# Yusheng-Xu/VGS-SVGS-Segmentation

Measured on AMD Instinct MI355X. Metric: segmented points/sec (end-to-end VGS), higher is better.
Workload: dtype f32

## Files before the change

### vgs-svgs-segmentation_amd/csrc/capi.hip

```cpp
#include <algorithm>
#include <cstdio>
#include <cstdlib>
#include <cstring>
#include <fstream>
#include <string>
#include <vector>

#include <dlfcn.h>

#include "vgs_context.hpp"

static thread_local std::string g_create_err;

static const char* const VGS_STAGE_NAMES[VGS_T_COUNT] = {"vgs:voxelize", "vgs:features", "vgs:adjacency", "vgs:localcut", "vgs:merge", "vgs:labels",
                                                         "vgs:total", "vgs:localcut_kernel", "vgs:supervoxels", "vgs:localcut_bulk", "", ""};
struct RoctxApi {
  int (*push)(const char*) = nullptr;
  int (*pop)() = nullptr;
  RoctxApi() {
    for (const char* name : {"librocprofiler-sdk-roctx.so.1", "librocprofiler-sdk-roctx.so", "libroctx64.so.4", "libroctx64.so"}) {
      void* h = dlopen(name, RTLD_LAZY | RTLD_LOCAL);
      if (!h) continue;
      push = (int (*)(const char*))dlsym(h, "roctxRangePushA");
      pop = (int (*)())dlsym(h, "roctxRangePop");
// ... 132 lines not shown
  }
  if (p->device < 0 || p->device >= ndev) { g_create_err = "vgs_create: bad device ordinal"; return VGS_E_ARG; }
  vgs_ctx* c = new (std::nothrow) vgs_ctx();
  if (!c) return VGS_E_NOMEM;
  c->P = *p;
  c->device = p->device;
  int prio_lo = 0, prio_hi = 0;
  if (hipSetDevice(c->device) != hipSuccess || hipStreamCreateWithFlags(&c->stream, hipStreamNonBlocking) != hipSuccess ||
      hipDeviceGetStreamPriorityRange(&prio_lo, &prio_hi) != hipSuccess ||
      hipStreamCreateWithPriority(&c->stream2, hipStreamNonBlocking, prio_hi) != hipSuccess ||
      hipStreamCreateWithPriority(&c->stream3, hipStreamNonBlocking, prio_hi) != hipSuccess ||
      hipStreamCreateWithPriority(&c->stream4, hipStreamNonBlocking, prio_hi) != hipSuccess) {
    g_create_err = "vgs_create: hipSetDevice/hipStreamCreate failed";
    vgs_destroy(c);
    return VGS_E_HIP;
  }
  if (hipHostMalloc(&c->pin, 4096, hipHostMallocDefault) != hipSuccess) c->pin = nullptr;
  bool ok = hipStreamCreateWithFlags(&c->s_h2d, hipStreamNonBlocking) == hipSuccess &&
            hipStreamCreateWithFlags(&c->s_d2h, hipStreamNonBlocking) == hipSuccess &&
            hipEventCreateWithFlags(&c->ev_h2d, hipEventDisableTiming) == hipSuccess &&
            hipEventCreateWithFlags(&c->ev_d2h, hipEventDisableTiming) == hipSuccess &&
            hipEventCreateWithFlags(&c->ev_rb, hipEventDisableTiming) == hipSuccess &&
            hipEventCreateWithFlags(&c->ev_ho, hipEventDisableTiming) == hipSuccess &&
            hipEventCreateWithFlags(&c->ev_ho2, hipEventDisableTiming) == hipSuccess;
  for (int i = 0; ok && i < 16; ++i) ok = hipEventCreate(&c->ev[i]) == hipSuccess;
  for (int i = 0; ok && i < VGS_T_COUNT; ++i) ok = hipEventCreate(&c->tev[i][0]) == hipSuccess && hipEventCreate(&c->tev[i][1]) == hipSuccess;
  if (!ok) { g_create_err = "vgs_create: hipStreamCreate/hipEventCreate failed"; vgs_destroy(c); return VGS_E_HIP; }
  vgs_read_env_knobs(c);
  *out = c;
  return VGS_OK;
}

void vgs_destroy(vgs_ctx* c) {
  if (!c) return;
  (void)hipSetDevice(c->device);
  if (c->stream) (void)hipStreamSynchronize(c->stream);
  if (c->stream2) (void)hipStreamSynchronize(c->stream2);
  if (c->stream3) (void)hipStreamSynchronize(c->stream3);
  if (c->stream4) (void)hipStreamSynchronize(c->stream4);
  if (c->s_h2d) (void)hipStreamSynchronize(c->s_h2d);
  if (c->s_d2h) (void)hipStreamSynchronize(c->s_d2h);
  c->xyz_buf[0].release(); c->xyz_buf[1].release(); c->pt_label_alt.release(); c->grow_state.release();
  c->code_a.release(); c->code_b.release(); c->perm_a.release(); c->perm_b.release(); c->sort_tmp.release();
  c->head_flag.release(); c->pt_vox.release(); c->vox_tile.release(); c->vox_code.release(); c->vox_start.release();
  c->xs.release(); c->ys.release(); c->zs.release();
  c->node.release(); c->used_ids.release(); c->used_rank.release();
  c->hkey.release(); c->hval.release(); c->offsets.release(); c->adj_masks.release(); c->adj_gtab.release(); c->adj_nvals.release(); c->adj_nrank.release(); c->adj_key.release(); c->adj_off.release(); c->adj_cnt.release(); c->adj_mused.release();
// ... 15 lines not shown
  c->ps_in.release(); c->ps_nnodes.release(); c->ps_key.release(); c->ps_val.release(); c->ps_seg.release(); c->ps_nn.release(); c->ps_tmp.release();
  c->ps_meta.release(); c->ps_part.release(); c->ps_d.release(); c->ps_f.release(); c->ps_npts.release();
  c->cl_off.release(); c->cl_idx.release(); c->conn.release(); c->evals.release(); c->lc_pending.release(); c->lc_defer.release(); c->lc_defer_flag.release(); c->csize.release(); c->attach.release(); c->cc_flags.release(); c->parent.release(); c->csz.release();
  c->vc_cen.release(); c->vc_nrm.release(); c->vc_dist.release(); c->vc_state.release(); c->vc_tile_start.release(); c->vc_cell.release(); c->vc_plive.release(); c->vc_tile_of.release(); c->vc_tchg.release(); c->vc_nbr_tiles.release(); c->vc_halo.release(); c->vc_tile_meta.release(); c->vc_pool.release(); c->vc_ring.release(); c->vc_dbg.release(); c->vc_label.release();
  c->vc_seedkey.release(); c->vc_sums.release(); c->vc_count.release(); c->vc_accu.release(); c->vc_alive.release();
  c->sv_label.release(); c->sv_key_a.release(); c->sv_key_b.release(); c->cell_code_a.release(); c->cell_code_b.release();
  c->cell_id_a.release(); c->cell_id_b.release(); c->cell_start.release();
  c->owned.release(); c->straddle.release(); c->mixsrc.release(); c->bnd_code.release(); c->bnd_root.release(); c->root_label.release();
  c->bnd_code2.release(); c->bnd_root2.release(); c->bnd_cnt.release(); c->broot.release();
  c->kept_rank.release(); c->vox_label.release(); c->pt_label.release(); c->counters.release(); c->work_ids.release();
  if (c->pin) (void)hipHostFree(c->pin);
  for (int i = 0; i < 16; ++i) if (c->ev[i]) (void)hipEventDestroy(c->ev[i]);
  for (int i = 0; i < VGS_T_COUNT; ++i) for (int k = 0; k < 2; ++k) if (c->tev[i][k]) (void)hipEventDestroy(c->tev[i][k]);
  if (c->stream) (void)hipStreamDestroy(c->stream);
  if (c->stream2) (void)hipStreamDestroy(c->stream2);
  if (c->stream3) (void)hipStreamDestroy(c->stream3);
  if (c->stream4) (void)hipStreamDestroy(c->stream4);
  if (c->s_h2d) (void)hipStreamDestroy(c->s_h2d);
  if (c->s_d2h) (void)hipStreamDestroy(c->s_d2h);
  if (c->ev_h2d) (void)hipEventDestroy(c->ev_h2d);
  if (c->ev_rb) (void)hipEventDestroy(c->ev_rb);
  if (c->ev_ho) (void)hipEventDestroy(c->ev_ho);
  if (c->ev_ho2) (void)hipEventDestroy(c->ev_ho2);
  if (c->ev_d2h) (void)hipEventDestroy(c->ev_d2h);
  delete c;
}

vgs_status vgs_set_params(vgs_ctx* c, const vgs_params* p) {
  if (!c || !p) return VGS_E_ARG;
  if (!(p->voxel_size > 0.f) || !(p->graph_size > 0.f) || !(p->sig_w != 0.f)) { c->err = "vgs_set_params: voxel_size, graph_size > 0, sig_w != 0"; return VGS_E_ARG; }
  if (p->method != c->P.method || p->device != c->P.device) { c->err = "vgs_set_params: method and device are fixed at vgs_create"; return VGS_E_ARG; }
  if (p->vccs_mode != 0 && p->vccs_mode != 1) { c->err = "vgs_set_params: vccs_mode must be 0 (synchronous variant) or 1 (PCL's order)"; return VGS_E_ARG; }
  int keep = ST_SEGMENTED;
  const vgs_params& o = c->P;
  if (p->cut_thred != o.cut_thred || p->sig_p != o.sig_p || p->sig_n != o.sig_n || p->sig_o != o.sig_o || p->sig_e != o.sig_e ||
      p->sig_c != o.sig_c || p->sig_w != o.sig_w || p->adjacency_min != o.adjacency_min || p->voxels_min != o.voxels_min ||
      p->q7_count_as_index != o.q7_count_as_index)
    keep = ST_ADJACENCY;
  if (p->graph_size != o.graph_size) keep = ST_FEATURES;
  if (p->points_min != o.points_min) keep = ST_VOXELS;
  if (p->voxel_size != o.voxel_size || p->seed_size != o.seed_size || p->color_impt != o.color_impt ||
      p->spatial_impt != o.spatial_impt || p->normal_impt != o.normal_impt || p->vccs_mode != o.vccs_mode)
    keep = ST_POINTS;
  if (c->stage > keep) c->stage = keep;
  if (keep < ST_SEGMENTED) { c->sd_valid = false; c->sb_valid[0] = c->sb_valid[1] = false; c->sg_valid = false; c->cmp_valid = false; c->rf_valid = false; c->cmp_own_cells = -1; c->sg_halo_valid = false; c->sg_own_K = -1; c->rf_halo_valid = false; c->rf_band_n = -1; }
  if (keep == ST_POINTS && c->P.method == 3 && !c->sv_labels_external) { c->sv_have_labels = false; c->sv_max_label = 0; c->sv_label_n = -1; }
// ... 549 lines not shown
```

### vgs-svgs-segmentation_amd/csrc/localcut.hip

```cpp
#include <algorithm>
#include <cmath>
#include <cstring>
#include <vector>
#include <cstdio>
#include <cstdlib>

#include "vgs_context.hpp"

#ifndef LC_TB
#define LC_TB 256
#endif
#ifndef LC_SMALL_CAP
#define LC_SMALL_CAP 4096
#endif
#define LC_NBIN 2048

#define LC_TBINS 64
struct LcParams {
  VgsWeightParams W;
  float cut;
  int prune_unused;
  float d2_stop;
  float ctab_scale;
  const float* ctab;
// ... 789 lines not shown
      const size_t sm = lc_smem_bytes<SMALL_M, SMALL_CAP, false>();
      VGS_HIP_TRY(c, hipFuncSetAttribute((const void*)kern, hipFuncAttributeMaxDynamicSharedMemorySize, (int)sm));
      hipLaunchKernelGGL(kern, dim3(nw), dim3(LC_TB), sm, strm, ids, arg_n, n_dev, c->adj_key.p, c->adj_cnt.p, c->adj_stride,
                         c->node.p, LP, c->conn.p, cnt, c->evals.p, (uint32_t*)nullptr);
    } else {
      auto kern = k_localcut<LARGE_M, LARGE_CAP, false>;
      const size_t sm = lc_smem_bytes<LARGE_M, LARGE_CAP, false>();
      VGS_HIP_TRY(c, hipFuncSetAttribute((const void*)kern, hipFuncAttributeMaxDynamicSharedMemorySize, (int)sm));
      hipLaunchKernelGGL(kern, dim3(nw), dim3(LC_TB), sm, strm, ids, arg_n, n_dev, c->adj_key.p, c->adj_cnt.p, c->adj_stride,
                         c->node.p, LP, c->conn.p, cnt, c->evals.p, ids_d );
    }
    return VGS_OK;
  };
  static_assert(WAVE_B <= SMALL_M, "wave-kernel hand-overs must fit the mid-size workgroup kernel");
  uint32_t* dbg_buf = nullptr;
#ifdef VGS_PROF
  VGS_HIP_TRY(c, s_dbg.ensure(4 * (size_t)U));
  VGS_HIP_TRY(c, hipMemset(s_dbg.p, 0, 16 * (size_t)U));
  dbg_buf = s_dbg.p;
#endif
  VGS_HIP_TRY(c, hipEventRecord(c->ev[6], c->stream));
  if (WP.dbg_stop != 0 || WP.shell0 < 0.0f) VGS_HIP_TRY(c, hipMemsetAsync(c->conn.p, 0, (size_t)U * c->adj_stride, c->stream));
  c->pl_enabled_at_launch = false;
  c->lc_tail.gated = false; c->lc_tail.pg_xl_queued = false;
  c->lc_tail.open = true; c->lc_tail.dense = dense; c->lc_tail.grid_f = 0; c->lc_tail.grid_g = GRID_G; c->lc_tail.tail_ms = 0.f;
  VGS_HIP_TRY(c, hipEventRecord(c->ev[2], c->stream));
  VGS_HIP_TRY(c, hipStreamWaitEvent(c->stream2, c->ev[2], 0));
  VGS_HIP_TRY(c, hipStreamWaitEvent(c->stream3, c->ev[2], 0));
  VGS_HIP_TRY(c, hipEventRecord(c->ev[9], c->stream3));
  VGS_HIP_TRY(c, hipStreamWaitEvent(c->stream, c->ev[9], 0));
  const unsigned int n_wide = nabc[2] + nabc[3] + nabc[5];
  bool pg_wide = c->pl_enabled && c->K.pg_wide != 0 && dense && n_wide > 0 && (uint64_t)n_wide * (uint64_t)c->K.pg_wide_frac > (uint64_t)U;
  if (pg_wide) {
    VGS_HIP_TRY(c, hipStreamWaitEvent(c->stream4, c->ev[2], 0));
    vgs_status sb = vgs_pairlists_build(c, c->stream2, nullptr, nullptr, nullptr, 0, true, LP.ctab, LP.ctab_scale, LP.d2_stop, 0, LcGate{nullptr, 0u}, true);
    if (sb != VGS_OK) return sb;
    pg_wide = c->pl_enabled;
  }
  if (pg_wide) {
    const PairLists PLw = {(const uint2*)c->pl_state.p, c->pl_ent.p, c->pl_state.p + (size_t)c->V * 9, c->pl_w_ring};
    const PgGeom G = {c->vox_code.p, c->P.voxel_size, (float)c->box.min[0], (float)c->box.min[1], (float)c->box.min[2], c->adj_r2};
    uint32_t* const wbits = c->cb_enabled ? c->conn_bits.p : (uint32_t*)nullptr;
    uint32_t* const ids_xl_pg = c->work_ids.p + (10 + LW_HO_BINS) * U;
    unsigned int* const d_nxl = (unsigned int*)(c->counters.p + 56);
    const bool pg_xl = c->cb_R <= 10 && !c->K.no_pg_xl && n_above_d != 0u;
    c->lc_tail.pg_xl_queued = pg_xl && nabc[3] > 0;
    VGS_HIP_TRY(c, hipEventRecord(c->ev_ho2, c->stream2));
// ... 125 lines not shown
  }
  VGS_HIP_TRY(c, hipStreamWaitEvent(c->stream, c->ev[8], 0));
  VGS_HIP_TRY(c, hipStreamWaitEvent(c->stream, c->ev[5], 0));
  if (nabc[3] + nabc[5] > 0) VGS_HIP_TRY(c, hipStreamWaitEvent(c->stream, c->ev[12], 0));
  if (c->K.no_overlap) {
    VGS_HIP_TRY(c, hipStreamWaitEvent(c->stream, c->ev[4], 0));
    VGS_HIP_TRY(c, hipStreamWaitEvent(c->stream, c->ev[3], 0));
    if (c->cb_enabled)
      hipLaunchKernelGGL(k_conn_bits, dim3((unsigned)U), dim3(64), 0, c->stream, c->lc_pending.p, U, c->adj_cnt.p, c->adj_stride, c->conn.p, c->adj_off.p,
                         c->cb_R, c->cb_words, c->conn_bits.p, CbLists{}, 0);
    VGS_HIP_TRY(c, hipMemsetAsync(c->lc_pending.p, 0, (size_t)U, c->stream));
  }
  if (c->pl_enabled_at_launch) c->lc_tail.gated = true;
  c->lc_tail.grid_f = grid_f;
  for (int k = 0; k < 5; ++k) c->lc_tail.nabc[k] = nabc[k];
  c->lc_tail.nabc[2] += nabc[5];
  VGS_HIP_TRY(c, hipEventRecord(c->ev[13], c->stream));
  c->counts[13] = nabc[0] + nabc[4]; c->counts[14] = nabc[1] + nabc[2] + nabc[5] + nabc[6]; c->counts[15] = nabc[3];
  c->counts[VGS_N_PAIRS] = -1;
  VGS_HIP_TRY(c, hipGetLastError());
  return VGS_OK;
}

vgs_status vgs_localcut_finish(vgs_ctx* c, unsigned int* n_deferred) {
  if (n_deferred) *n_deferred = 0;
  if (!c->lc_tail.open) return VGS_OK;
  c->lc_tail.open = false;
  const int64_t U = c->U;
  unsigned long long* cnt = (unsigned long long*)c->counters.p;
  const unsigned int grid_f = c->lc_tail.grid_f, GRID_G = c->lc_tail.grid_g;
  uint32_t* ids_f = c->work_ids.p + 8 * U;
  uint32_t* ids_g = c->work_ids.p + 5 * U;
  LcParams LP;
  LP.W = make_weight_params(c->P);
  LP.cut = c->P.cut_thred;
  LP.prune_unused = 0;
  LP.xl_from = c->K.dbg_xl_from;
  LP.dbg_max_m = c->K.dbg_max_m;
  {
    const float reach = 2.0f * c->P.graph_size + 4.0f * c->P.voxel_size;
    LP.d2_stop = lc_d2_stop(LP.W, LP.cut, reach * reach * 1.01f);
    LP.ctab = c->lc_ctab.p; LP.ctab_scale = c->lc_ctab_scale;
  }
  constexpr int SMALL_M = 128, SMALL_CAP = LC_SMALL_CAP;
  constexpr int LARGE_M = 2048, LARGE_CAP = 8192;
  constexpr int XL_M = 8192, XL_CAP = 4096;
  uint32_t* ids_xl = c->work_ids.p + 3 * U;
  auto launch_rest = [&](const uint32_t* ids, unsigned int nw, bool mid) -> vgs_status {
    if (nw == 0) return VGS_OK;
    if (mid) {
      auto kern = k_localcut<SMALL_M, SMALL_CAP, false>;
      const size_t sm = lc_smem_bytes<SMALL_M, SMALL_CAP, false>();
      VGS_HIP_TRY(c, hipFuncSetAttribute((const void*)kern, hipFuncAttributeMaxDynamicSharedMemorySize, (int)sm));
      hipLaunchKernelGGL(kern, dim3(nw), dim3(LC_TB), sm, c->stream, ids, (int)nw, (const unsigned int*)nullptr, c->adj_key.p, c->adj_cnt.p,
                         c->adj_stride, c->node.p, LP, c->conn.p, cnt, c->evals.p, (uint32_t*)nullptr);
    } else {
      auto kern = k_localcut<LARGE_M, LARGE_CAP, false>;
      const size_t sm = lc_smem_bytes<LARGE_M, LARGE_CAP, false>();
      VGS_HIP_TRY(c, hipFuncSetAttribute((const void*)kern, hipFuncAttributeMaxDynamicSharedMemorySize, (int)sm));
      hipLaunchKernelGGL(kern, dim3(nw), dim3(LC_TB), sm, c->stream, ids, (int)nw, (const unsigned int*)nullptr, c->adj_key.p, c->adj_cnt.p,
                         c->adj_stride, c->node.p, LP, c->conn.p, cnt, c->evals.p, ids_xl);
    }
    return VGS_OK;
  };
  VGS_HIP_TRY(c, hipStreamWaitEvent(c->stream, c->ev[4], 0));
  VGS_HIP_TRY(c, hipStreamWaitEvent(c->stream, c->ev[3], 0));
  VGS_HIP_TRY(c, hipEventRecord(c->ev[7], c->stream));
  unsigned long long hc[64] = {0};
  VGS_READBACK(c, hc, cnt, sizeof(hc));
  const unsigned long long lc_why[4] = {hc[3], hc[4], hc[5], hc[6]};
  if (!c->lc_tail.pg_xl_queued && (unsigned int)(hc[56] & 0xffffffffull) != 0u) { c->err = "local cut: voxels queued for a kernel that was not launched"; return VGS_E_STATE; }
  c->lc_tail.many = c->lc_tail.gated && (unsigned int)(hc[57] & 0xffffffffull) == LC_MANY;
  c->lc_diag[9] = (int64_t)hc[63]; c->lc_diag[10] = (int64_t)(hc[58] & 0xffffffffull); c->lc_diag[11] = (int64_t)hc[62]; c->lc_diag[12] = (int64_t)hc[60];
  const unsigned long long* h = hc;
  const unsigned int nfg[2] = {(unsigned int)((hc[14] & 0xffffffffull) + (hc[14] >> 32) + (hc[15] & 0xffffffffull) + (hc[15] >> 32)),
                               (unsigned int)(hc[11] >> 32)};
  const unsigned int nf = nfg[0] + nfg[1];
  if (n_deferred) *n_deferred = (unsigned int)(hc[13] & 0xffffffffull);
  const bool dense = c->lc_tail.dense;
  const unsigned int nf2 = (unsigned int)(hc[12] & 0xffffffffull), ng2 = (unsigned int)(hc[12] >> 32);
  {
    vgs_status st = VGS_OK;
    bool more = false;
    if (dense) {
      if (nf2 > 0) { st = launch_rest(c->work_ids.p + 7 * U, nf2, true); more = true; }
      if (st == VGS_OK && ng2 > 0) { st = launch_rest(c->work_ids.p + 4 * U, ng2, false); more = true; }
    } else {
      if (nfg[0] > grid_f) { st = launch_rest(ids_f + grid_f, nfg[0] - grid_f, true); more = true; }
      if (st == VGS_OK && nfg[1] > GRID_G) { st = launch_rest(ids_g + GRID_G, nfg[1] - GRID_G, false); more = true; }
    }
    if (st != VGS_OK) return st;
    if (more) {
      VGS_HIP_TRY(c, hipEventRecord(c->ev[7], c->stream));
      VGS_HIP_TRY(c, hipMemcpyAsync(hc, cnt, 8 * sizeof(unsigned long long), hipMemcpyDeviceToHost, c->stream));
      VGS_HIP_TRY(c, hipStreamSynchronize(c->stream));
    }
  }
  c->lc_diag[8] = 0;
  if (hc[1] > 0) {
    static_assert(XL_M <= 65535 && XL_M >= 8192, "pair ids are 2 x 16 bits; a row holds at most 8192 ball offsets");
    const unsigned int n_xl = (unsigned int)hc[1];
    if ((int64_t)n_xl > U) { c->err = "local cut: corrupt overflow count"; return VGS_E_HIP; }
    auto kern = k_localcut<XL_M, XL_CAP, false>;
    const size_t sm = lc_smem_bytes<XL_M, XL_CAP, false>();
    VGS_HIP_TRY(c, hipFuncSetAttribute((const void*)kern, hipFuncAttributeMaxDynamicSharedMemorySize, (int)sm));
    VGS_HIP_TRY(c, hipMemsetAsync(cnt + 1, 0, sizeof(unsigned long long), c->stream));
    hipLaunchKernelGGL(kern, dim3(n_xl), dim3(LC_TB), sm, c->stream, ids_xl, (int)n_xl, (const unsigned int*)nullptr, c->adj_key.p, c->adj_cnt.p,
                       c->adj_stride, c->node.p, LP, c->conn.p, cnt, c->evals.p, (uint32_t*)nullptr);
    VGS_HIP_TRY(c, hipGetLastError());
    VGS_HIP_TRY(c, hipEventRecord(c->ev[7], c->stream));
    VGS_HIP_TRY(c, hipMemcpyAsync(hc, cnt, 8 * sizeof(unsigned long long), hipMemcpyDeviceToHost, c->stream));
    VGS_HIP_TRY(c, hipStreamSynchronize(c->stream));
    c->lc_diag[8] = (int64_t)n_xl;
  }
  if (c->cb_enabled && nf > 0) {
    CbLists L;
    const unsigned int nb4[4] = {(unsigned int)(hc[14] & 0xffffffffull), (unsigned int)(hc[14] >> 32), (unsigned int)(hc[15] & 0xffffffffull), (unsigned int)(hc[15] >> 32)};
    unsigned int at = 0;
    for (int k = 0; k < 4; ++k) { L.ids[k] = ids_f + (size_t)k * U; at += nb4[k]; L.end[k] = at; }
    L.ids[4] = ids_g; at += nfg[1]; L.end[4] = at;
    hipLaunchKernelGGL(k_conn_bits, dim3(at), dim3(64), 0, c->stream, c->lc_pending.p, U, c->adj_cnt.p, c->adj_stride, c->conn.p, c->adj_off.p,
                       c->cb_R, c->cb_words, c->conn_bits.p, L, 1);
    VGS_HIP_TRY(c, hipGetLastError());
  }
  c->counts[VGS_N_REATTACHED + 2] = nf;
  c->lc_diag[0] = (int64_t)lc_why[0]; c->lc_diag[1] = (int64_t)(lc_why[1] + lc_why[2] + lc_why[3]); c->lc_diag[2] = (int64_t)nfg[0]; c->lc_diag[3] = (int64_t)nf2 + (int64_t)ng2;
  c->lc_diag[4] = (int64_t)nfg[1]; c->lc_diag[5] = (int64_t)h[1]; c->lc_diag[6] = (int64_t)(hc[13] & 0xffffffffull); c->lc_diag[7] = (int64_t)h[0];
  VGS_HIP_TRY(c, hipGetLastError());
  float kms = 0.f;
  VGS_HIP_TRY(c, hipEventElapsedTime(&kms, c->ev[6], c->ev[7]));
  c->times[VGS_T_LOCALCUT_KERNEL] = kms;
  VGS_HIP_TRY(c, hipEventElapsedTime(&kms, c->ev[10], c->ev[11]));
  c->times[VGS_T_LOCALCUT_BULK] = kms;
  if (hipEventElapsedTime(&kms, c->ev[13], c->ev[7]) == hipSuccess && kms > 0.f) c->lc_tail.tail_ms = kms;
  if (c->K.debug && nfg[0] > 0) {
    std::vector<uint32_t> idf(nfg[0]), ev((size_t)U), ac((size_t)U);
    {
      const unsigned int nb4[4] = {(unsigned int)(hc[14] & 0xffffffffull), (unsigned int)(hc[14] >> 32), (unsigned int)(hc[15] & 0xffffffffull), (unsigned int)(hc[15] >> 32)};
      size_t at = 0;
      for (int k = 0; k < 4; ++k) {
        if (nb4[k]) VGS_HIP_TRY(c, hipMemcpy(idf.data() + at, ids_f + (size_t)k * U, (size_t)nb4[k] * 4, hipMemcpyDeviceToHost));
        at += nb4[k];
      }
    }
// ... 78 lines not shown
```

### vgs-svgs-segmentation_amd/csrc/merge.hip

```cpp
#include <cstring>
#include <string.h>
#include <utility>

#include <rocprim/rocprim.hpp>

#include "vgs_context.hpp"

struct MgParams {
  VgsWeightParams W;
  int adjacency_min;
  int q7;
  int64_t V;
};

#define MF_CAP_TRIPS 8
template <int W, int T>
__device__ __forceinline__ void mf_load(const uint8_t* __restrict__ flags, int limit, int k0, int sub, uint8_t (&f)[T]) {
#pragma unroll
  for (int q = 0; q < T; ++q) {
    const int k = k0 + q * W + sub;
    f[q] = flags[k < limit ? k : 0];
  }
}
template <int W, int T>
// ... 477 lines not shown
  uint8_t* mutual = nullptr;
  unsigned int n_cand = 0, n_succ = 0;
  bool compressed = false, united = false;
  if (U > 0) {
    if (c->conn.cap < 2 * (size_t)U * c->adj_stride) { c->err = "connect buffer missing (local cut stage not run)"; return VGS_E_STATE; }
    mutual = c->conn.p + (size_t)U * c->adj_stride;
    const uint16_t* gt = (c->P.method == 2 && c->adj_have_gtab) ? c->adj_gtab.p : nullptr;
    const float inv_res2 = 1.0f / (c->P.voxel_size * c->P.voxel_size);
    if (c->have_region) { vgs_status so = vgs_compute_owned(c); if (so != VGS_OK) return so; }
    const uint8_t* owned_early = c->have_region ? c->owned.p : (const uint8_t*)nullptr;
    unsigned int* d_ndefer = (unsigned int*)(c->counters.p + 13);
    const bool early_union = c->lc_tail.open && !c->K.no_overlap;
    if (early_union) VGS_HIP_TRY(c, c->lc_defer_flag.ensure((size_t)U));
    const bool use_bits = c->cb_enabled && c->P.method == 2 && c->adj_have_off;
    const uint16_t* cb_off = use_bits ? c->adj_off.p : (const uint16_t*)nullptr;
    const int cb_lut = c->cb_R;
    const uint32_t* cb_bits = use_bits ? c->conn_bits.p : (const uint32_t*)nullptr;
    const LcGate g_first = {(c->lc_tail.open && c->lc_tail.gated) ? (const unsigned int*)(c->counters.p + 57) : (const unsigned int*)nullptr, LC_FEW};
    const size_t first_lds = (c->lc_tail.open && c->K.cross_lds_kb > 0) ? (size_t)c->K.cross_lds_kb * 1024 : 0;
    hipLaunchKernelGGL(k_cross, dim3(vgs_xcd_grid((U + CX_ROWS - 1) / CX_ROWS)), dim3(64), first_lds, c->stream, c->used_ids.p, c->used_rank.p, U, c->adj_key.p, c->adj_cnt.p,
                       c->adj_stride, c->conn.p, mutual, c->csize.p, c->parent.p, gt, c->adj_gstride, c->adj_nrank.p, inv_res2,
                       c->lc_tail.open ? c->lc_pending.p : (const uint8_t*)nullptr, c->lc_defer.p, d_ndefer, (const uint32_t*)nullptr, 0,
                       cb_off, cb_lut, cb_bits, c->cb_words, early_union ? c->lc_defer_flag.p : (uint8_t*)nullptr, g_first, owned_early);
    if (early_union) {
      hipLaunchKernelGGL(k_compress, dim3(nbV), dim3(TB), 0, c->stream, c->parent.p, V);
      hipLaunchKernelGGL(k_union_mutual, dim3((unsigned)((U + UM_ROWS - 1) / UM_ROWS)), dim3(64), first_lds, c->stream, c->used_ids.p, U, c->adj_key.p, c->adj_cnt.p,
                         c->adj_stride, mutual, c->attach.p, owned_early, c->parent.p, 0, c->lc_defer_flag.p, (const uint32_t*)nullptr, 0, g_first);
      compressed = true; united = true;
    }
    unsigned int n_defer = 0;
    {
      vgs_status sf = vgs_localcut_finish(c, &n_defer);
      if (sf != VGS_OK) return sf;
    }
    if (c->lc_tail.many) {
      hipLaunchKernelGGL(k_merge_init, dim3(nbV), dim3(TB), 0, c->stream, c->parent.p, c->csize.p, c->attach.p, c->cc_flags.p, c->csz.p, V);
      hipLaunchKernelGGL(k_cross, dim3(vgs_xcd_grid((U + CX_ROWS - 1) / CX_ROWS)), dim3(64), 0, c->stream, c->used_ids.p, c->used_rank.p, U, c->adj_key.p, c->adj_cnt.p,
                         c->adj_stride, c->conn.p, mutual, c->csize.p, c->parent.p, gt, c->adj_gstride, c->adj_nrank.p, inv_res2,
                         (const uint8_t*)nullptr, c->lc_defer.p, d_ndefer, (const uint32_t*)nullptr, 0, cb_off, cb_lut, cb_bits, c->cb_words, (uint8_t*)nullptr,
                         LcGate{nullptr, 0u}, owned_early);
      compressed = false; united = false;
      n_defer = 0;
    }
    if (n_defer > 0) {
      hipLaunchKernelGGL(k_cross, dim3((n_defer + CX_ROWS - 1) / CX_ROWS), dim3(64), 0, c->stream, c->used_ids.p, c->used_rank.p, U, c->adj_key.p, c->adj_cnt.p,
                         c->adj_stride, c->conn.p, mutual, c->csize.p, early_union ? (uint32_t*)nullptr : c->parent.p, gt, c->adj_gstride, c->adj_nrank.p, inv_res2,
                         (const uint8_t*)nullptr, c->lc_defer.p, d_ndefer, c->lc_defer.p, (int)n_defer, cb_off, cb_lut, cb_bits, c->cb_words, (uint8_t*)nullptr, LcGate{nullptr, 0u});
      if (early_union)
        hipLaunchKernelGGL(k_union_mutual, dim3((n_defer + UM_ROWS - 1) / UM_ROWS), dim3(64), 0, c->stream, c->used_ids.p, U, c->adj_key.p, c->adj_cnt.p,
                           c->adj_stride, mutual, c->attach.p, owned_early, c->parent.p, 0, (const uint8_t*)nullptr, c->lc_defer.p, (int)n_defer, LcGate{nullptr, 0u});
    }
    VGS_HIP_TRY(c, c->work_ids.ensure((size_t)U + 16));
    unsigned int* d_ncand = (unsigned int*)(mcnt + 0);
    unsigned int* d_changed = (unsigned int*)(mcnt + 1);
    hipLaunchKernelGGL(k_cc_candidates, dim3((unsigned)((U + TB - 1) / TB)), dim3(TB), 0, c->stream, c->used_ids.p, U, c->adj_mused.p,
                       c->csize.p, MP.adjacency_min, c->cc_flags.p, c->work_ids.p, d_ncand);
    const bool hide = !c->have_region && vgs_can_split_readback(c) && !early_union;
    if (hide) {
      vgs_status sb = vgs_readback_begin(c, d_ncand, 4);
      if (sb != VGS_OK) return sb;
      hipLaunchKernelGGL(k_compress, dim3(nbV), dim3(TB), 0, c->stream, c->parent.p, V);
      compressed = true;
      vgs_status se = vgs_readback_end(c, &n_cand, 4);
      if (se != VGS_OK) return se;
    } else {
      VGS_READBACK(c, &n_cand, d_ncand, 4);
    }
    if (n_cand > 0) {
      unsigned int* d_chg4 = (unsigned int*)(mcnt + 4);
      for (int round = 0; round < 1 << 18; ++round) {
        VGS_HIP_TRY(c, hipMemsetAsync(d_chg4, 0, 16, c->stream));
        for (int q = 0; q < 4; ++q)
          hipLaunchKernelGGL((k_cc_pass<false>), dim3(n_cand), dim3(64), 0, c->stream, c->work_ids.p, (int)n_cand, c->used_ids.p,
                             c->adj_key.p, c->adj_cnt.p, c->adj_mused.p, c->adj_stride, c->node.p, c->csize.p, c->cc_flags.p, MP, c->attach.p, d_chg4 + q);
        unsigned int ch = 0;
        if (hide && !united) {
          vgs_status sb = vgs_readback_begin(c, d_chg4 + 3, 4);
          if (sb != VGS_OK) return sb;
          hipLaunchKernelGGL(k_union_mutual, dim3((unsigned)((U + UM_ROWS - 1) / UM_ROWS)), dim3(64), 0, c->stream, c->used_ids.p, U, c->adj_key.p, c->adj_cnt.p,
                             c->adj_stride, mutual, c->attach.p, (const uint8_t*)nullptr, c->parent.p, 0, (const uint8_t*)nullptr, (const uint32_t*)nullptr, 0, LcGate{nullptr, 0u});
          united = true;
          vgs_status se = vgs_readback_end(c, &ch, 4);
          if (se != VGS_OK) return se;
        } else {
          VGS_READBACK(c, &ch, d_chg4 + 3, 4);
        }
        if (!ch) break;
      }
      hipLaunchKernelGGL((k_cc_pass<true>), dim3(n_cand), dim3(64), 0, c->stream, c->work_ids.p, (int)n_cand, c->used_ids.p, c->adj_key.p,
                         c->adj_cnt.p, c->adj_mused.p, c->adj_stride, c->node.p, c->csize.p, c->cc_flags.p, MP, c->attach.p, d_changed);
    }
  } else {
    VGS_HIP_TRY(c, c->conn.ensure(16));
  }
  if (c->have_region && U == 0) { vgs_status so = vgs_compute_owned(c); if (so != VGS_OK) return so; }
  if (U > 0 && !compressed) hipLaunchKernelGGL(k_compress, dim3(nbV), dim3(TB), 0, c->stream, c->parent.p, V);
  if (U > 0 && !united)
    hipLaunchKernelGGL(k_union_mutual, dim3((unsigned)((U + UM_ROWS - 1) / UM_ROWS)), dim3(64), 0, c->stream, c->used_ids.p, U, c->adj_key.p, c->adj_cnt.p,
                       c->adj_stride, mutual, c->attach.p, c->have_region ? c->owned.p : nullptr, c->parent.p, 1, (const uint8_t*)nullptr, (const uint32_t*)nullptr, 0, LcGate{nullptr, 0u});
  else if (U > 0 && n_cand > 0)
    hipLaunchKernelGGL(k_union_attach, dim3((n_cand + TB - 1) / TB), dim3(TB), 0, c->stream, c->work_ids.p, (int)n_cand, c->used_ids.p, c->attach.p, c->parent.p,
                       c->have_region ? c->owned.p : (const uint8_t*)nullptr);
  hipLaunchKernelGGL(k_flatten, dim3(nbV), dim3(TB), 0, c->stream, c->parent.p, V, c->have_region ? c->owned.p : nullptr, c->csz.p);
  VGS_HIP_TRY(c, hipEventRecord(c->ev[14], c->stream));
  uint32_t* keep_flag = c->head_flag.p;
  VGS_HIP_TRY(c, c->head_flag.ensure(V + 1));
  keep_flag = c->head_flag.p;
  unsigned int* d_nroots = (unsigned int*)(mcnt + 2);
  hipLaunchKernelGGL(k_root_flags, dim3((unsigned)((V + 1023) / 1024)), dim3(1024), 0, c->stream, c->parent.p, c->csz.p, V, c->P.method == 3 ? -1 : c->P.voxels_min,
                     keep_flag, d_nroots);
  size_t bytes = 0;
  VGS_HIP_TRY(c, rocprim::exclusive_scan(nullptr, bytes, keep_flag, c->kept_rank.p, 0u, (size_t)V, rocprim::plus<uint32_t>(), c->stream));
  VGS_HIP_TRY(c, c->sort_tmp.ensure(bytes));
// ... 22 lines not shown
```

### vgs-svgs-segmentation_amd/csrc/vgs_context.hpp

```cpp
#ifndef VGS_CONTEXT_HPP_
#define VGS_CONTEXT_HPP_

#include <hip/hip_runtime.h>
#include <stdint.h>
#include <string.h>

#include <string>
#include <vector>

#include "../../include/vgs.h"
#include "vgs_math.h"
#include "pairlist.hpp"

typedef VgsNode NodeRec;
static_assert(sizeof(NodeRec) == 64, "NodeRec must be 64 bytes");

#ifdef __HIPCC__
__device__ __forceinline__ int64_t vgs_xcd_item(unsigned int b, int64_t n) {
  const int64_t per = (n + 7) >> 3;
  return (int64_t)(b & 7u) * per + (int64_t)(b >> 3);
}
#endif
static inline unsigned int vgs_xcd_grid(int64_t n) { return (unsigned int)(((n + 7) >> 3) << 3); }

// ... 148 lines not shown
  DevBuf<uint64_t> adj_key;
  DevBuf<uint16_t> adj_off;
  bool adj_have_off = false;
  DevBuf<uint32_t> conn_bits;
  int cb_words = 0, cb_R = 0;
  bool cb_enabled = false;
  DevBuf<uint32_t> adj_cnt, adj_mused;
  bool adj_pruned = false;
  float adj_r2 = 0.f;

  DevBuf<uint8_t> nl_cnt;
  DevBuf<uint32_t> nl_tot;
  DevBuf<float4> nl_ent;
  bool nl_enabled = false;
  int nl_reach_steps = 0;
  bool nl_direct = false;

  DevBuf<uint8_t> pl_state;
  DevBuf<float4> pl_ent;
  DevBuf<uint32_t> pl_work;
  bool pl_enabled = false;
  bool pl_enabled_at_launch = false;
  hipEvent_t ev_ho = nullptr, ev_ho2 = nullptr;
  float pl_w_ring = 0.0f;

  DevBuf<uint8_t> conn;
  DevBuf<uint32_t> evals;
  DevBuf<uint8_t> lc_pending;
  DevBuf<uint8_t> lc_defer_flag;
  DevBuf<uint32_t> lc_defer;
  struct { bool open = false; bool dense = true; bool gated = false;  bool many = false;  unsigned int grid_f = 0, grid_g = 0, nabc[5] = {0, 0, 0, 0, 0}; float tail_ms = 0.f; bool pg_xl_queued = false;  } lc_tail;
  int64_t lc_diag[16] = {0};
  DevBuf<float> lc_ctab;
  float lc_ctab_key[8] = {0}, lc_ctab_scale = 0.0f;
  bool lc_ctab_valid = false;
  DevBuf<uint32_t> csize;
  DevBuf<int32_t> attach;
  DevBuf<uint8_t> cc_flags;
  DevBuf<uint32_t> parent;
  DevBuf<uint32_t> csz, kept_rank;
  DevBuf<int32_t> vox_label;
  DevBuf<int32_t> pt_label;
  DevBuf<int32_t> pt_label_alt;
  DevBuf<int64_t> cl_off;
  DevBuf<int32_t> cl_idx;
  bool cl_valid = false;
  DevBuf<uint32_t> sd_key, sd_ids, sd_vp, sd_seg;
  DevBuf<uint8_t> sd_tmp;
  DevBuf<double> sd_part;
  DevBuf<int64_t> sd_npts;
  DevBuf<int32_t> sd_nnodes;
  DevBuf<float> sd_bbox, sd_eig8;
  DevBuf<double> sd_cen, sd_cov, sd_eval, sd_evec;
  bool sd_valid = false;
// ... 100 lines not shown
};

#define VGS_HIP_TRY(ctx, expr)                                                                       \
  do {                                                                                               \
    hipError_t _e = (expr);                                                                          \
    if (_e != hipSuccess) {                                                                          \
      (ctx)->err = std::string(#expr) + ": " + hipGetErrorString(_e);                                \
      if (_e == hipErrorOutOfMemory) { (void)hipGetLastError(); return VGS_E_NOMEM; }                \
      return VGS_E_HIP;                                                                              \
    }                                                                                                \
  } while (0)

static inline vgs_status vgs_readback(vgs_ctx* c, void* dst, const void* src_dev, size_t bytes) {
  if (bytes > 4096 || !c->pin) {
    VGS_HIP_TRY(c, hipMemcpyAsync(dst, src_dev, bytes, hipMemcpyDeviceToHost, c->stream));
    VGS_HIP_TRY(c, hipStreamSynchronize(c->stream));
    return VGS_OK;
  }
  VGS_HIP_TRY(c, hipMemcpyAsync(c->pin, src_dev, bytes, hipMemcpyDeviceToHost, c->stream));
  VGS_HIP_TRY(c, hipStreamSynchronize(c->stream));
  memcpy(dst, c->pin, bytes);
  return VGS_OK;
}
#define VGS_CB_MAX_WORDS 624
#ifdef __HIPCC__
__device__ __forceinline__ uint32_t vgs_cb_index(uint32_t p, int R) {
  const int D = 2 * R + 1;
  const int dx = (int)(p & 31u) - 16 + R, dy = (int)((p >> 5) & 31u) - 16 + R, dz = (int)((p >> 10) & 31u) - 16 + R;
  return (uint32_t)((dz * D + dy) * D + dx);
}
#endif
#define VGS_READBACK(ctx, dst, src, bytes) do { vgs_status _s = vgs_readback((ctx), (dst), (src), (bytes)); if (_s != VGS_OK) return _s; } while (0)

static inline vgs_status vgs_readback_begin(vgs_ctx* c, const void* src_dev, size_t bytes) {
  if (bytes > 2048 || !c->pin || !c->ev_rb) return VGS_E_ARG;
  VGS_HIP_TRY(c, hipMemcpyAsync((char*)c->pin + 2048, src_dev, bytes, hipMemcpyDeviceToHost, c->stream));
  VGS_HIP_TRY(c, hipEventRecord(c->ev_rb, c->stream));
  return VGS_OK;
}
static inline vgs_status vgs_readback_end(vgs_ctx* c, void* dst, size_t bytes) {
  VGS_HIP_TRY(c, hipEventSynchronize(c->ev_rb));
  memcpy(dst, (char*)c->pin + 2048, bytes);
  return VGS_OK;
}
static inline bool vgs_can_split_readback(const vgs_ctx* c) { return c->pin != nullptr && c->ev_rb != nullptr; }

#define SD_TB 256
#define SD_PPT 8
#define SD_CHUNK (SD_TB * SD_PPT)
struct SdPrep { uint32_t *ids, *vp, *seg_node, *seg_chunk; int64_t n_chunks_max; };
vgs_status sd_prepare(vgs_ctx* c, int64_t K, SdPrep& o);
vgs_status sd_own_anchor(vgs_ctx* c, int64_t K, const SdPrep& P);
static inline bool vgs_is_tile(const vgs_ctx* c) { return c->have_region || c->n_own >= 0; }
#ifdef __HIPCC__
__device__ __forceinline__ int64_t vgs_find_voxel(const uint64_t* __restrict__ vox_code, int64_t V, uint64_t q) {
// ... 33 lines not shown
  uint32_t l = 0, h = m - 1;
  while (l < h) { const uint32_t mid = (l + h + 1) >> 1; if (s_vp[mid] <= q) l = mid; else h = mid - 1; }
  return q + s_dl[l];
}
#endif

vgs_status vgs_cut_order(vgs_ctx* c, std::vector<uint16_t>& ord_host, std::vector<uint32_t>& k_host, bool want_lists = false,
                         const uint8_t* list_flag = nullptr, std::vector<uint32_t>* list_cnt = nullptr, std::vector<int32_t>* list_ids = nullptr);
void vgs_read_env_knobs(vgs_ctx* c);

vgs_status vgs_stage_voxelize(vgs_ctx* c);
vgs_status vgs_stage_features(vgs_ctx* c);
vgs_status vgs_stage_adjacency(vgs_ctx* c);
vgs_status vgs_run_adjacency(vgs_ctx* c, bool full, uint64_t* out_key, uint32_t* out_cnt, uint32_t* out_nall, float r2, const uint32_t* ids = nullptr,
                             int64_t n_ids = 0);
bool vgs_unused_are_inert(const vgs_params& p);
vgs_status vgs_stage_nearlists(vgs_ctx* c);
vgs_status vgs_pairlists_begin(vgs_ctx* c, hipStream_t strm);
vgs_status vgs_pairlists_build(vgs_ctx* c, hipStream_t strm, const uint32_t* const* ids, const unsigned int* const* n_dev, const unsigned int* n_host,
                               int n_lists, bool all_rows, const float* ctab, float ctab_scale, float d2_stop, int slot, const LcGate& gate,
                               bool big_rows_too);
vgs_status vgs_stage_localcut(vgs_ctx* c);
vgs_status vgs_ensure_point_labels(vgs_ctx* c);
vgs_status vgs_localcut_finish(vgs_ctx* c, unsigned int* n_deferred);
vgs_status vgs_stage_merge(vgs_ctx* c);
vgs_status vgs_clusters_on_device(vgs_ctx* c);
vgs_status vgs_segdesc_on_device(vgs_ctx* c);
vgs_status vgs_segbox_on_device(vgs_ctx* c, int frame);
void sb_launch_frames(vgs_ctx* c, const double* evec, const double* cov, int64_t K, int frame, double* out);
vgs_status vgs_check_label_range(vgs_ctx* c, const char* fn, const int32_t* labels_dev, int64_t n, int64_t K);
vgs_status vgs_upload_point_labels(vgs_ctx* c, const int32_t* labels_host, int64_t n, const int32_t** labels_dev);
vgs_status vgs_seggraph_on_device(vgs_ctx* c);
vgs_status vgs_halo_find(vgs_ctx* c, const uint64_t* code_dev, const int32_t* label_dev, int64_t n, int32_t* halo_dev);
vgs_status vgs_refine_on_device(vgs_ctx* c, const vgs_refine_params& rp, int64_t* counts4);
vgs_status vgs_refine_own_on_device(vgs_ctx* c, const vgs_refine_params& rp, int64_t* counts5);
vgs_status vgs_stage_vccs(vgs_ctx* c);
vgs_status vgs_stage_svgs_group(vgs_ctx* c);
vgs_status vgs_stage_svgs_neighbours(vgs_ctx* c);
vgs_status vgs_grow_box_from(vgs_ctx* c, OctreeBox& box, bool record_epochs);
vgs_status vgs_compute_owned(vgs_ctx* c);

#endif
```

Baseline: 1.656 billion.

## Fork local-cut tail and CC passes onto a side stream during early union

When early union is active, the merge stage forks onto stream3 with an event. There it queues the local-cut counter readback and the tail local-cut kernels, and the deferred cross and connected-component passes follow on the same side stream. Meanwhile compress and union_mutual run on the main stream, and join events reconnect the two streams before dependent work. This aims to overlap the host readback latency and tail kernels with the union kernels, at the cost of extra event synchronisation and a risk of races on shared buffers such as parent and attach.

```diff
diff --git a/vgs-svgs-segmentation_amd/csrc/capi.hip b/vgs-svgs-segmentation_amd/csrc/capi.hip
--- a/vgs-svgs-segmentation_amd/csrc/capi.hip
+++ b/vgs-svgs-segmentation_amd/csrc/capi.hip
@@ -178,7 +178,9 @@
             hipEventCreateWithFlags(&c->ev_d2h, hipEventDisableTiming) == hipSuccess &&
             hipEventCreateWithFlags(&c->ev_rb, hipEventDisableTiming) == hipSuccess &&
             hipEventCreateWithFlags(&c->ev_ho, hipEventDisableTiming) == hipSuccess &&
-            hipEventCreateWithFlags(&c->ev_ho2, hipEventDisableTiming) == hipSuccess;
+            hipEventCreateWithFlags(&c->ev_ho2, hipEventDisableTiming) == hipSuccess &&
+            hipEventCreateWithFlags(&c->ev_fork, hipEventDisableTiming) == hipSuccess &&
+            hipEventCreateWithFlags(&c->ev_join, hipEventDisableTiming) == hipSuccess;
   for (int i = 0; ok && i < 16; ++i) ok = hipEventCreate(&c->ev[i]) == hipSuccess;
   for (int i = 0; ok && i < VGS_T_COUNT; ++i) ok = hipEventCreate(&c->tev[i][0]) == hipSuccess && hipEventCreate(&c->tev[i][1]) == hipSuccess;
   if (!ok) { g_create_err = "vgs_create: hipStreamCreate/hipEventCreate failed"; vgs_destroy(c); return VGS_E_HIP; }
@@ -240,6 +242,8 @@
   if (c->ev_rb) (void)hipEventDestroy(c->ev_rb);
   if (c->ev_ho) (void)hipEventDestroy(c->ev_ho);
   if (c->ev_ho2) (void)hipEventDestroy(c->ev_ho2);
+  if (c->ev_fork) (void)hipEventDestroy(c->ev_fork);
+  if (c->ev_join) (void)hipEventDestroy(c->ev_join);
   if (c->ev_d2h) (void)hipEventDestroy(c->ev_d2h);
   delete c;
 }
diff --git a/vgs-svgs-segmentation_amd/csrc/localcut.hip b/vgs-svgs-segmentation_amd/csrc/localcut.hip
--- a/vgs-svgs-segmentation_amd/csrc/localcut.hip
+++ b/vgs-svgs-segmentation_amd/csrc/localcut.hip
@@ -835,7 +835,7 @@
   VGS_HIP_TRY(c, hipEventRecord(c->ev[6], c->stream));
   if (WP.dbg_stop != 0 || WP.shell0 < 0.0f) VGS_HIP_TRY(c, hipMemsetAsync(c->conn.p, 0, (size_t)U * c->adj_stride, c->stream));
   c->pl_enabled_at_launch = false;
-  c->lc_tail.gated = false; c->lc_tail.pg_xl_queued = false;
+  c->lc_tail.gated = false; c->lc_tail.pg_xl_queued = false; c->lc_tail.rb_queued = false;
   c->lc_tail.open = true; c->lc_tail.dense = dense; c->lc_tail.grid_f = 0; c->lc_tail.grid_g = GRID_G; c->lc_tail.tail_ms = 0.f;
   VGS_HIP_TRY(c, hipEventRecord(c->ev[2], c->stream));
   VGS_HIP_TRY(c, hipStreamWaitEvent(c->stream2, c->ev[2], 0));
@@ -1007,7 +1007,17 @@
   return VGS_OK;
 }
 
-vgs_status vgs_localcut_finish(vgs_ctx* c, unsigned int* n_deferred) {
+vgs_status vgs_localcut_finish_queue(vgs_ctx* c, hipStream_t s) {
+  if (!c->lc_tail.open || !c->pin || c->lc_tail.rb_queued) return VGS_OK;
+  VGS_HIP_TRY(c, hipStreamWaitEvent(s, c->ev[4], 0));
+  VGS_HIP_TRY(c, hipStreamWaitEvent(s, c->ev[3], 0));
+  VGS_HIP_TRY(c, hipEventRecord(c->ev[7], s));
+  VGS_HIP_TRY(c, hipMemcpyAsync(c->pin, c->counters.p, 64 * sizeof(unsigned long long), hipMemcpyDeviceToHost, s));
+  c->lc_tail.rb_queued = true;
+  return VGS_OK;
+}
+
+vgs_status vgs_localcut_finish(vgs_ctx* c, hipStream_t s, unsigned int* n_deferred) {
   if (n_deferred) *n_deferred = 0;
   if (!c->lc_tail.open) return VGS_OK;
   c->lc_tail.open = false;
@@ -1037,22 +1047,28 @@
       auto kern = k_localcut<SMALL_M, SMALL_CAP, false>;
       const size_t sm = lc_smem_bytes<SMALL_M, SMALL_CAP, false>();
       VGS_HIP_TRY(c, hipFuncSetAttribute((const void*)kern, hipFuncAttributeMaxDynamicSharedMemorySize, (int)sm));
-      hipLaunchKernelGGL(kern, dim3(nw), dim3(LC_TB), sm, c->stream, ids, (int)nw, (const unsigned int*)nullptr, c->adj_key.p, c->adj_cnt.p,
+      hipLaunchKernelGGL(kern, dim3(nw), dim3(LC_TB), sm, s, ids, (int)nw, (const unsigned int*)nullptr, c->adj_key.p, c->adj_cnt.p,
                          c->adj_stride, c->node.p, LP, c->conn.p, cnt, c->evals.p, (uint32_t*)nullptr);
     } else {
       auto kern = k_localcut<LARGE_M, LARGE_CAP, false>;
       const size_t sm = lc_smem_bytes<LARGE_M, LARGE_CAP, false>();
       VGS_HIP_TRY(c, hipFuncSetAttribute((const void*)kern, hipFuncAttributeMaxDynamicSharedMemorySize, (int)sm));
-      hipLaunchKernelGGL(kern, dim3(nw), dim3(LC_TB), sm, c->stream, ids, (int)nw, (const unsigned int*)nullptr, c->adj_key.p, c->adj_cnt.p,
+      hipLaunchKernelGGL(kern, dim3(nw), dim3(LC_TB), sm, s, ids, (int)nw, (const unsigned int*)nullptr, c->adj_key.p, c->adj_cnt.p,
                          c->adj_stride, c->node.p, LP, c->conn.p, cnt, c->evals.p, ids_xl);
     }
     return VGS_OK;
   };
-  VGS_HIP_TRY(c, hipStreamWaitEvent(c->stream, c->ev[4], 0));
-  VGS_HIP_TRY(c, hipStreamWaitEvent(c->stream, c->ev[3], 0));
-  VGS_HIP_TRY(c, hipEventRecord(c->ev[7], c->stream));
   unsigned long long hc[64] = {0};
-  VGS_READBACK(c, hc, cnt, sizeof(hc));
+  if (c->lc_tail.rb_queued) {
+    c->lc_tail.rb_queued = false;
+    VGS_HIP_TRY(c, hipStreamSynchronize(s));
+    memcpy(hc, c->pin, sizeof(hc));
+  } else {
+    VGS_HIP_TRY(c, hipStreamWaitEvent(s, c->ev[4], 0));
+    VGS_HIP_TRY(c, hipStreamWaitEvent(s, c->ev[3], 0));
+    VGS_HIP_TRY(c, hipEventRecord(c->ev[7], s));
+    VGS_READBACK_ON(c, s, hc, cnt, sizeof(hc));
+  }
   const unsigned long long lc_why[4] = {hc[3], hc[4], hc[5], hc[6]};
   if (!c->lc_tail.pg_xl_queued && (unsigned int)(hc[56] & 0xffffffffull) != 0u) { c->err = "local cut: voxels queued for a kernel that was not launched"; return VGS_E_STATE; }
   c->lc_tail.many = c->lc_tail.gated && (unsigned int)(hc[57] & 0xffffffffull) == LC_MANY;
@@ -1076,9 +1092,9 @@
     }
     if (st != VGS_OK) return st;
     if (more) {
-      VGS_HIP_TRY(c, hipEventRecord(c->ev[7], c->stream));
-      VGS_HIP_TRY(c, hipMemcpyAsync(hc, cnt, 8 * sizeof(unsigned long long), hipMemcpyDeviceToHost, c->stream));
-      VGS_HIP_TRY(c, hipStreamSynchronize(c->stream));
+      VGS_HIP_TRY(c, hipEventRecord(c->ev[7], s));
+      VGS_HIP_TRY(c, hipMemcpyAsync(hc, cnt, 8 * sizeof(unsigned long long), hipMemcpyDeviceToHost, s));
+      VGS_HIP_TRY(c, hipStreamSynchronize(s));
     }
   }
   c->lc_diag[8] = 0;
@@ -1089,13 +1105,13 @@
     auto kern = k_localcut<XL_M, XL_CAP, false>;
     const size_t sm = lc_smem_bytes<XL_M, XL_CAP, false>();
     VGS_HIP_TRY(c, hipFuncSetAttribute((const void*)kern, hipFuncAttributeMaxDynamicSharedMemorySize, (int)sm));
-    VGS_HIP_TRY(c, hipMemsetAsync(cnt + 1, 0, sizeof(unsigned long long), c->stream));
-    hipLaunchKernelGGL(kern, dim3(n_xl), dim3(LC_TB), sm, c->stream, ids_xl, (int)n_xl, (const unsigned int*)nullptr, c->adj_key.p, c->adj_cnt.p,
+    VGS_HIP_TRY(c, hipMemsetAsync(cnt + 1, 0, sizeof(unsigned long long), s));
+    hipLaunchKernelGGL(kern, dim3(n_xl), dim3(LC_TB), sm, s, ids_xl, (int)n_xl, (const unsigned int*)nullptr, c->adj_key.p, c->adj_cnt.p,
                        c->adj_stride, c->node.p, LP, c->conn.p, cnt, c->evals.p, (uint32_t*)nullptr);
     VGS_HIP_TRY(c, hipGetLastError());
-    VGS_HIP_TRY(c, hipEventRecord(c->ev[7], c->stream));
-    VGS_HIP_TRY(c, hipMemcpyAsync(hc, cnt, 8 * sizeof(unsigned long long), hipMemcpyDeviceToHost, c->stream));
-    VGS_HIP_TRY(c, hipStreamSynchronize(c->stream));
+    VGS_HIP_TRY(c, hipEventRecord(c->ev[7], s));
+    VGS_HIP_TRY(c, hipMemcpyAsync(hc, cnt, 8 * sizeof(unsigned long long), hipMemcpyDeviceToHost, s));
+    VGS_HIP_TRY(c, hipStreamSynchronize(s));
     c->lc_diag[8] = (int64_t)n_xl;
   }
   if (c->cb_enabled && nf > 0) {
@@ -1104,7 +1120,7 @@
     unsigned int at = 0;
     for (int k = 0; k < 4; ++k) { L.ids[k] = ids_f + (size_t)k * U; at += nb4[k]; L.end[k] = at; }
     L.ids[4] = ids_g; at += nfg[1]; L.end[4] = at;
-    hipLaunchKernelGGL(k_conn_bits, dim3(at), dim3(64), 0, c->stream, c->lc_pending.p, U, c->adj_cnt.p, c->adj_stride, c->conn.p, c->adj_off.p,
+    hipLaunchKernelGGL(k_conn_bits, dim3(at), dim3(64), 0, s, c->lc_pending.p, U, c->adj_cnt.p, c->adj_stride, c->conn.p, c->adj_off.p,
                        c->cb_R, c->cb_words, c->conn_bits.p, L, 1);
     VGS_HIP_TRY(c, hipGetLastError());
   }
diff --git a/vgs-svgs-segmentation_amd/csrc/merge.hip b/vgs-svgs-segmentation_amd/csrc/merge.hip
--- a/vgs-svgs-segmentation_amd/csrc/merge.hip
+++ b/vgs-svgs-segmentation_amd/csrc/merge.hip
@@ -523,7 +523,12 @@
                        c->adj_stride, c->conn.p, mutual, c->csize.p, c->parent.p, gt, c->adj_gstride, c->adj_nrank.p, inv_res2,
                        c->lc_tail.open ? c->lc_pending.p : (const uint8_t*)nullptr, c->lc_defer.p, d_ndefer, (const uint32_t*)nullptr, 0,
                        cb_off, cb_lut, cb_bits, c->cb_words, early_union ? c->lc_defer_flag.p : (uint8_t*)nullptr, g_first, owned_early);
+    hipStream_t s = c->stream;
     if (early_union) {
+      VGS_HIP_TRY(c, hipEventRecord(c->ev_fork, c->stream));
+      VGS_HIP_TRY(c, hipStreamWaitEvent(c->stream3, c->ev_fork, 0));
+      s = c->stream3;
+      { vgs_status sq = vgs_localcut_finish_queue(c, s); if (sq != VGS_OK) return sq; }
       hipLaunchKernelGGL(k_compress, dim3(nbV), dim3(TB), 0, c->stream, c->parent.p, V);
       hipLaunchKernelGGL(k_union_mutual, dim3((unsigned)((U + UM_ROWS - 1) / UM_ROWS)), dim3(64), first_lds, c->stream, c->used_ids.p, U, c->adj_key.p, c->adj_cnt.p,
                          c->adj_stride, mutual, c->attach.p, owned_early, c->parent.p, 0, c->lc_defer_flag.p, (const uint32_t*)nullptr, 0, g_first);
@@ -531,10 +536,15 @@
     }
     unsigned int n_defer = 0;
     {
-      vgs_status sf = vgs_localcut_finish(c, &n_defer);
+      vgs_status sf = vgs_localcut_finish(c, s, &n_defer);
       if (sf != VGS_OK) return sf;
     }
     if (c->lc_tail.many) {
+      if (s != c->stream) {
+        VGS_HIP_TRY(c, hipEventRecord(c->ev_join, s));
+        VGS_HIP_TRY(c, hipStreamWaitEvent(c->stream, c->ev_join, 0));
+        s = c->stream;
+      }
       hipLaunchKernelGGL(k_merge_init, dim3(nbV), dim3(TB), 0, c->stream, c->parent.p, c->csize.p, c->attach.p, c->cc_flags.p, c->csz.p, V);
       hipLaunchKernelGGL(k_cross, dim3(vgs_xcd_grid((U + CX_ROWS - 1) / CX_ROWS)), dim3(64), 0, c->stream, c->used_ids.p, c->used_rank.p, U, c->adj_key.p, c->adj_cnt.p,
                          c->adj_stride, c->conn.p, mutual, c->csize.p, c->parent.p, gt, c->adj_gstride, c->adj_nrank.p, inv_res2,
@@ -544,9 +554,13 @@
       n_defer = 0;
     }
     if (n_defer > 0) {
-      hipLaunchKernelGGL(k_cross, dim3((n_defer + CX_ROWS - 1) / CX_ROWS), dim3(64), 0, c->stream, c->used_ids.p, c->used_rank.p, U, c->adj_key.p, c->adj_cnt.p,
+      hipLaunchKernelGGL(k_cross, dim3((n_defer + CX_ROWS - 1) / CX_ROWS), dim3(64), 0, s, c->used_ids.p, c->used_rank.p, U, c->adj_key.p, c->adj_cnt.p,
                          c->adj_stride, c->conn.p, mutual, c->csize.p, early_union ? (uint32_t*)nullptr : c->parent.p, gt, c->adj_gstride, c->adj_nrank.p, inv_res2,
                          (const uint8_t*)nullptr, c->lc_defer.p, d_ndefer, c->lc_defer.p, (int)n_defer, cb_off, cb_lut, cb_bits, c->cb_words, (uint8_t*)nullptr, LcGate{nullptr, 0u});
+      if (s != c->stream) {
+        VGS_HIP_TRY(c, hipEventRecord(c->ev_fork, s));
+        VGS_HIP_TRY(c, hipStreamWaitEvent(c->stream, c->ev_fork, 0));
+      }
       if (early_union)
         hipLaunchKernelGGL(k_union_mutual, dim3((n_defer + UM_ROWS - 1) / UM_ROWS), dim3(64), 0, c->stream, c->used_ids.p, U, c->adj_key.p, c->adj_cnt.p,
                            c->adj_stride, mutual, c->attach.p, owned_early, c->parent.p, 0, (const uint8_t*)nullptr, c->lc_defer.p, (int)n_defer, LcGate{nullptr, 0u});
@@ -554,7 +568,7 @@
     VGS_HIP_TRY(c, c->work_ids.ensure((size_t)U + 16));
     unsigned int* d_ncand = (unsigned int*)(mcnt + 0);
     unsigned int* d_changed = (unsigned int*)(mcnt + 1);
-    hipLaunchKernelGGL(k_cc_candidates, dim3((unsigned)((U + TB - 1) / TB)), dim3(TB), 0, c->stream, c->used_ids.p, U, c->adj_mused.p,
+    hipLaunchKernelGGL(k_cc_candidates, dim3((unsigned)((U + TB - 1) / TB)), dim3(TB), 0, s, c->used_ids.p, U, c->adj_mused.p,
                        c->csize.p, MP.adjacency_min, c->cc_flags.p, c->work_ids.p, d_ncand);
     const bool hide = !c->have_region && vgs_can_split_readback(c) && !early_union;
     if (hide) {
@@ -565,14 +579,14 @@
       vgs_status se = vgs_readback_end(c, &n_cand, 4);
       if (se != VGS_OK) return se;
     } else {
-      VGS_READBACK(c, &n_cand, d_ncand, 4);
+      VGS_READBACK_ON(c, s, &n_cand, d_ncand, 4);
     }
     if (n_cand > 0) {
       unsigned int* d_chg4 = (unsigned int*)(mcnt + 4);
       for (int round = 0; round < 1 << 18; ++round) {
-        VGS_HIP_TRY(c, hipMemsetAsync(d_chg4, 0, 16, c->stream));
+        VGS_HIP_TRY(c, hipMemsetAsync(d_chg4, 0, 16, s));
         for (int q = 0; q < 4; ++q)
-          hipLaunchKernelGGL((k_cc_pass<false>), dim3(n_cand), dim3(64), 0, c->stream, c->work_ids.p, (int)n_cand, c->used_ids.p,
+          hipLaunchKernelGGL((k_cc_pass<false>), dim3(n_cand), dim3(64), 0, s, c->work_ids.p, (int)n_cand, c->used_ids.p,
                              c->adj_key.p, c->adj_cnt.p, c->adj_mused.p, c->adj_stride, c->node.p, c->csize.p, c->cc_flags.p, MP, c->attach.p, d_chg4 + q);
         unsigned int ch = 0;
         if (hide && !united) {
@@ -584,12 +598,16 @@
           vgs_status se = vgs_readback_end(c, &ch, 4);
           if (se != VGS_OK) return se;
         } else {
-          VGS_READBACK(c, &ch, d_chg4 + 3, 4);
+          VGS_READBACK_ON(c, s, &ch, d_chg4 + 3, 4);
         }
         if (!ch) break;
       }
-      hipLaunchKernelGGL((k_cc_pass<true>), dim3(n_cand), dim3(64), 0, c->stream, c->work_ids.p, (int)n_cand, c->used_ids.p, c->adj_key.p,
+      hipLaunchKernelGGL((k_cc_pass<true>), dim3(n_cand), dim3(64), 0, s, c->work_ids.p, (int)n_cand, c->used_ids.p, c->adj_key.p,
                          c->adj_cnt.p, c->adj_mused.p, c->adj_stride, c->node.p, c->csize.p, c->cc_flags.p, MP, c->attach.p, d_changed);
+    }
+    if (s != c->stream) {
+      VGS_HIP_TRY(c, hipEventRecord(c->ev_join, s));
+      VGS_HIP_TRY(c, hipStreamWaitEvent(c->stream, c->ev_join, 0));
     }
   } else {
     VGS_HIP_TRY(c, c->conn.ensure(16));
diff --git a/vgs-svgs-segmentation_amd/csrc/vgs_context.hpp b/vgs-svgs-segmentation_amd/csrc/vgs_context.hpp
--- a/vgs-svgs-segmentation_amd/csrc/vgs_context.hpp
+++ b/vgs-svgs-segmentation_amd/csrc/vgs_context.hpp
@@ -194,6 +194,7 @@
   bool pl_enabled = false;
   bool pl_enabled_at_launch = false;
   hipEvent_t ev_ho = nullptr, ev_ho2 = nullptr;
+  hipEvent_t ev_fork = nullptr, ev_join = nullptr;
   float pl_w_ring = 0.0f;
 
   DevBuf<uint8_t> conn;
@@ -201,7 +202,7 @@
   DevBuf<uint8_t> lc_pending;
   DevBuf<uint8_t> lc_defer_flag;
   DevBuf<uint32_t> lc_defer;
-  struct { bool open = false; bool dense = true; bool gated = false;  bool many = false;  unsigned int grid_f = 0, grid_g = 0, nabc[5] = {0, 0, 0, 0, 0}; float tail_ms = 0.f; bool pg_xl_queued = false;  } lc_tail;
+  struct { bool open = false; bool dense = true; bool gated = false;  bool many = false;  unsigned int grid_f = 0, grid_g = 0, nabc[5] = {0, 0, 0, 0, 0}; float tail_ms = 0.f; bool pg_xl_queued = false;  bool rb_queued = false;  } lc_tail;
   int64_t lc_diag[16] = {0};
   DevBuf<float> lc_ctab;
   float lc_ctab_key[8] = {0}, lc_ctab_scale = 0.0f;
@@ -348,6 +349,17 @@
   memcpy(dst, c->pin, bytes);
   return VGS_OK;
 }
+static inline vgs_status vgs_readback_on(vgs_ctx* c, hipStream_t s, void* dst, const void* src_dev, size_t bytes) {
+  if (bytes > 2048 || !c->pin) {
+    VGS_HIP_TRY(c, hipMemcpyAsync(dst, src_dev, bytes, hipMemcpyDeviceToHost, s));
+    VGS_HIP_TRY(c, hipStreamSynchronize(s));
+    return VGS_OK;
+  }
+  VGS_HIP_TRY(c, hipMemcpyAsync(c->pin, src_dev, bytes, hipMemcpyDeviceToHost, s));
+  VGS_HIP_TRY(c, hipStreamSynchronize(s));
+  memcpy(dst, c->pin, bytes);
+  return VGS_OK;
+}
 #define VGS_CB_MAX_WORDS 624
 #ifdef __HIPCC__
 __device__ __forceinline__ uint32_t vgs_cb_index(uint32_t p, int R) {
@@ -357,6 +369,7 @@
 }
 #endif
 #define VGS_READBACK(ctx, dst, src, bytes) do { vgs_status _s = vgs_readback((ctx), (dst), (src), (bytes)); if (_s != VGS_OK) return _s; } while (0)
+#define VGS_READBACK_ON(ctx, s, dst, src, bytes) do { vgs_status _s = vgs_readback_on((ctx), (s), (dst), (src), (bytes)); if (_s != VGS_OK) return _s; } while (0)
 
 static inline vgs_status vgs_readback_begin(vgs_ctx* c, const void* src_dev, size_t bytes) {
   if (bytes > 2048 || !c->pin || !c->ev_rb) return VGS_E_ARG;
@@ -436,7 +449,8 @@
                                bool big_rows_too);
 vgs_status vgs_stage_localcut(vgs_ctx* c);
 vgs_status vgs_ensure_point_labels(vgs_ctx* c);
-vgs_status vgs_localcut_finish(vgs_ctx* c, unsigned int* n_deferred);
+vgs_status vgs_localcut_finish_queue(vgs_ctx* c, hipStream_t s);
+vgs_status vgs_localcut_finish(vgs_ctx* c, hipStream_t s, unsigned int* n_deferred);
 vgs_status vgs_stage_merge(vgs_ctx* c);
 vgs_status vgs_clusters_on_device(vgs_ctx* c);
 vgs_status vgs_segdesc_on_device(vgs_ctx* c);
```

New measurement: 1.682 billion, median of 6. 1.02x the previous value.
